# lyndonchan/wsss-analysis

Hardware: AMD Instinct MI355X
Metric: images/sec CAM+CRF pseudo-labels, VOC2012 321x321 (higher is better)
Workload: dtype f16x3; 1 GPU; resnet50 CAM + dense-CRF (M=21, 10 mean-field iters), 321x321, batch 32 images (=64 samples) per GPU, image-sharded; batch_images=32, num_classes=20, parallelism=image-sharded x1, no collective, steps_per_rank=239

## Files before the change

### wsss-analysis_amd/csrc/crf.hip

```cpp
#include "common.h"

#include <atomic>
#include <cmath>
#include <cstring>
#include <memory>

namespace {

constexpr unsigned long long EMPTY_KEY = 0xFFFFFFFFFFFFFFFFull;
typedef float f32x2_t __attribute__((ext_vector_type(2)));

struct LatticeDev {
    int d = 0;
    int rep = 1;
    int rows = 0;
    int32_t *offset = nullptr;
    float *bary = nullptr;
    float *norm = nullptr;
    int2 *nbr = nullptr;
    int32_t *tslot_start = nullptr;
    int2 *slot_desc = nullptr;
    float *tent_w = nullptr;
    uint8_t *tent_p = nullptr;
    int32_t *row_slot_start = nullptr;
    int n_tiles = 0, n_slots = 0;
    bool sorted_dest = false;
    long long n_pix = 0;
    int M_cur = 0;
    float alpha = 0.f;
    int32_t *tile_rows = nullptr;
    int2 *tile_pstart = nullptr;
    int32_t *tile_list = nullptr;
    int n_tiles_occ = 0;
    int4 *gt_cnt = nullptr;
    int2 *gt_rows = nullptr;
    uint4 *gt_nbr = nullptr;
    uint4 *gt_pix = nullptr;
    int gt_stride = 0;
    std::vector<int32_t> v_per_image;
    int32_t *img_row = nullptr;
    int max_img_rows = 0;
    uint32_t *part_row = nullptr;
    bool bl_ok = false;
    int2 *bl_blk = nullptr;
    int bl_cap = 0;
    mutable std::vector<int2> bl_blk_host;
    mutable int bl_M = -1, bl_nblk = 0;
    mutable size_t bl_lds = 0;
};

constexpr int TILE_W = 16, TILE_H = 16, TILE_PIX = TILE_W * TILE_H;
static_assert(TILE_PIX <= 256, "an entry's pixel index is stored in one byte");
constexpr int SLOT_ENT = 32;
constexpr int SORT_MAX = 2048;
static_assert(TILE_PIX * 6 <= SORT_MAX && SORT_MAX <= 65535, "tile too large for the in-LDS grouping");

struct TileGeom {
    int H, W, ntx, nty, tpi;
};
__host__ __device__ inline TileGeom make_geom(int H, int W) {
    TileGeom g;
    g.H = H; g.W = W;
    g.ntx = (W + TILE_W - 1) / TILE_W;
    g.nty = (H + TILE_H - 1) / TILE_H;
    g.tpi = g.ntx * g.nty;
    return g;
}
struct TileBox {
    int x0, y0, cw, ch;
    int ebase;
};
__host__ __device__ inline TileBox tile_box(const TileGeom &g, int j) {
// ... 765 lines not shown
                                                                 float *__restrict__ tent_w, const uint8_t *__restrict__ tent_p) {
    const int tile = blockIdx.x;
    const int b = tile / tg.tpi, j = tile - b * tg.tpi;
    const TileBox tb = tile_box(tg, j);
    const int N = tg.H * tg.W;
    const int ne = tb.cw * tb.ch * dp1;
    const long long ebase = ((long long)b * N + tb.ebase) * dp1;
    const unsigned cw_magic = tile_div_magic(tb.cw);
    for (int i = threadIdx.x; i < ne; i += 256) {
        const int t = (int)tent_p[ebase + i];
        const int ty = (int)(((unsigned)t * cw_magic) >> 16), tx = t - ty * tb.cw;
        const long long p = (long long)b * N + (long long)(tb.y0 + ty) * tg.W + tb.x0 + tx;
        tent_w[ebase + i] = tent_w[ebase + i] * norm[p];
    }
}

template <int D>
__global__ void neighbors_kernel(const unsigned long long *__restrict__ rowkey, const int32_t *__restrict__ rowimg,
                                 const unsigned long long *__restrict__ table, const int32_t *__restrict__ slot2row,
                                 long long cap, unsigned cap_mask, int rows, int2 *__restrict__ nbr) {
    const int j = blockIdx.y;
    long long rbeg, rend;
    xcd_range(rows, rbeg, rend);
    for (int row = (int)rbeg + (int)threadIdx.x; row < (int)rend; row += (int)blockDim.x) {
        const long long i = (long long)j * rows + row;
        int *nb = reinterpret_cast<int *>(nbr);
        if (row == 0) {
            nb[2 * i] = 0;
            continue;
        }
        int key[D], k1[D];
        unpack_key<D>(rowkey[row], key);
#pragma unroll
        for (int k = 0; k < D; ++k) k1[k] = key[k] - 1;
        if (j < D) {
#pragma unroll
            for (int k = 0; k < D; ++k)
                if (k == j) k1[k] = key[k] + D;
        }
        const int b = rowimg[row];
        const unsigned long long *tb = table + (long long)b * cap;
        const int32_t *s2r = slot2row + (long long)b * cap;
        unsigned long long p1;
        int r1 = 0;
        if (pack_key<D>(k1, p1)) {
            const int s = hash_lookup(tb, cap_mask, p1);
            if (s >= 0) r1 = s2r[s];
        }
        nb[2 * i] = r1;
        if (r1 > 0) nb[2 * ((long long)j * rows + r1) + 1] = row;
    }
}


constexpr float PFIX_SCALE = 16777216.0f;
constexpr float PFIX_INV = 1.0f / 16777216.0f;
static_assert(SLOT_ENT * 2.5f < 127.0f, "slot partials must fit the 2^24 fixed-point int32");

template <bool PLAIN>
__device__ __forceinline__ f32x4_t combine_slots4(const f32x4_t *__restrict__ part, int sb, int se, unsigned LP, unsigned l) {
    f32x4_t first = part[(unsigned)sb * LP + l];
    if (se - sb == 1) return first;
    if (PLAIN) {
        for (int i = sb + 1; i < se; ++i) {
            const f32x4_t v = part[(unsigned)i * LP + l];
#pragma unroll
            for (int k = 0; k < 4; ++k) first[k] += v[k];
        }
        return first;
    }
    long long acc[4] = {0, 0, 0, 0};
    for (int i = sb; i < se; i += 4) {
        f32x4_t v[4];
#pragma unroll
        for (int u = 0; u < 4; ++u) v[u] = part[(unsigned)min(i + u, se - 1) * LP + l];
#pragma unroll
        for (int u = 0; u < 4; ++u)
            if (i + u < se) {
#pragma unroll
                for (int k = 0; k < 4; ++k) acc[k] += (long long)__float2int_rn(v[u][k] * PFIX_SCALE);
            }
    }
    f32x4_t o = {(float)acc[0] * PFIX_INV, (float)acc[1] * PFIX_INV, (float)acc[2] * PFIX_INV, (float)acc[3] * PFIX_INV};
    return o;
}

__global__ __launch_bounds__(256) void slot_ones_kernel(const int32_t *__restrict__ tslot_start, const int2 *__restrict__ slot_desc,
                                                        const float *__restrict__ tent_w, int dp1, TileGeom tg,
                                                        float *__restrict__ part) {
    const int tile = blockIdx.x;
    const int b = tile / tg.tpi, j = tile - b * tg.tpi;
    const TileBox tb = tile_box(tg, j);
    const long long ebase = ((long long)b * tg.H * tg.W + tb.ebase) * dp1;
    __shared__ float w[TILE_PIX * 6];
    const int ne = tb.cw * tb.ch * dp1;
    {
        constexpr int EN = (TILE_PIX * 6 + 255) / 256;
        float ew[EN];
#pragma unroll
        for (int k = 0; k < EN; ++k) {
            const int i = (int)threadIdx.x + k * 256;
            ew[k] = i < ne ? tent_w[ebase + i] : 0.f;
        }
#pragma unroll
        for (int k = 0; k < EN; ++k) {
            const int i = (int)threadIdx.x + k * 256;
            if (i < ne) w[i] = ew[k];
        }
    }
    __syncthreads();
    for (int s = tslot_start[tile] + threadIdx.x; s < tslot_start[tile + 1]; s += 256) {
        const int2 d = slot_desc[s];
        const int i0 = d.x & 0xffff, n = d.x >> 16;
        float acc = 0.f;
        for (int i = 0; i < n; ++i) acc += w[i0 + i];
        part[d.y] = acc;
    }
}
__global__ void combine1_kernel(const float *__restrict__ part, const int32_t *__restrict__ row_slot_start, int rows,
                                float *__restrict__ val) {
    for (int row = blockIdx.x * blockDim.x + threadIdx.x; row < rows; row += gridDim.x * blockDim.x) {
        long long acc = 0;
        for (int i = row_slot_start[row]; i < row_slot_start[row + 1]; ++i)
            acc += (long long)__float2int_rn(part[i] * PFIX_SCALE);
        val[row] = (float)acc * PFIX_INV;
    }
}

__global__ __launch_bounds__(256) void combine4_kernel(const f32x4_t *__restrict__ part, const int32_t *__restrict__ row_slot_start,
                                                       int LP, int rows_local, int n_slots, int rep, f32x4_t *__restrict__ val) {
    const int rpb = 256 / LP;
    const int tr = threadIdx.x / LP;
    const int l = threadIdx.x - tr * LP;
    if (tr >= rpb) return;
    long long rbeg, rend;
    int rk;
    xcd_range_rep(rows_local, rep, rk, rbeg, rend);
    part += (size_t)rk * n_slots * LP;
    val += (size_t)rk * rows_local * LP;
    for (long long row = rbeg + tr; row < rend; row += rpb) {
        const int sb = row_slot_start[row], se = row_slot_start[row + 1];
        f32x4_t o = {0.f, 0.f, 0.f, 0.f};
        if (se > sb) o = combine_slots4<true>(part, sb, se, (unsigned)LP, (unsigned)l);
        val[(unsigned)row * (unsigned)LP + l] = o;
    }
}

constexpr int CB_ROWS = 32;
__global__ __launch_bounds__(256) void combine4_balanced_kernel(const f32x4_t *__restrict__ part, const int32_t *__restrict__ row_slot_start,
                                                                const uint32_t *__restrict__ part_row, int LP, int rows,
                                                                f32x4_t *__restrict__ val) {
    __shared__ int rss_l[CB_ROWS + 1];
    __shared__ unsigned long long acc[CB_ROWS * 32];
    const int r0 = blockIdx.x * CB_ROWS;
    const int nr = min(CB_ROWS, rows - r0);
    const int P0 = row_slot_start[r0], P1 = row_slot_start[r0 + nr];
    for (int i = threadIdx.x; i <= nr; i += 256) rss_l[i] = row_slot_start[r0 + i];
    for (int i = threadIdx.x; i < CB_ROWS * 32; i += 256) acc[i] = 0ull;
    const int gpb = 256 / LP;
    const int tr = threadIdx.x / LP, l = threadIdx.x - tr * LP;
    constexpr int U = 4;
    f32x4_t v[U];
    uint32_t pr[U];
    auto fetch = [&](int p) {
#pragma unroll
        for (int u = 0; u < U; ++u) {
            const int pp = p + u * gpb;
            v[u] = f32x4_t{0.f, 0.f, 0.f, 0.f};
            pr[u] = 0u;
            if (tr < gpb && pp < P1) {
                v[u] = part[(unsigned)pp * (unsigned)LP + l];
                if (part_row) pr[u] = part_row[pp];
            }
        }
    };
    fetch(P0 + tr);
    __syncthreads();
    if (tr < gpb) {
        for (int p = P0 + tr; p < P1; p += U * gpb) {
            if (p != P0 + tr) fetch(p);
#pragma unroll
            for (int u = 0; u < U; ++u) {
                const int pp = p + u * gpb;
                if (pp < P1) {
                    int lo;
                    bool single;
                    if (part_row) {
                        lo = (int)(pr[u] & 0xffffffu) - r0;
                        single = (pr[u] >> 24) == 1u;
                    } else {
                        lo = 0;
                        int hi = nr;
                        while (hi - lo > 1) {
                            const int mid = (lo + hi) >> 1;
                            if (rss_l[mid] <= pp) lo = mid;
                            else hi = mid;
                        }
                        single = rss_l[lo + 1] - rss_l[lo] == 1;
                    }
                    if (single) {
                        val[(unsigned)(r0 + lo) * (unsigned)LP + l] = v[u];
                    } else {
#pragma unroll
                        for (int k = 0; k < 4; ++k)
                            atomicAdd(&acc[lo * 32 + 4 * l + k], (unsigned long long)(long long)__float2int_rn(v[u][k] * PFIX_SCALE));
                    }
                }
            }
        }
    }
    __syncthreads();
    if (tr < gpb) {
        for (int row = tr; row < nr; row += gpb) {
            const int n = rss_l[row + 1] - rss_l[row];
            if (n == 1) continue;
            f32x4_t o = {0.f, 0.f, 0.f, 0.f};
            if (n > 1) {
#pragma unroll
                for (int k = 0; k < 4; ++k) o[k] = (float)(long long)acc[row * 32 + 4 * l + k] * PFIX_INV;
            }
            val[(unsigned)(r0 + row) * (unsigned)LP + l] = o;
        }
    }
}


__global__ __launch_bounds__(256) void blur1_kernel(const float *__restrict__ in, const int2 *__restrict__ nbr,
                                                    int rows, float *__restrict__ out) {
    for (int row = blockIdx.x * blockDim.x + threadIdx.x; row < rows; row += gridDim.x * blockDim.x) {
        const int2 nb = nbr[row];
        out[row] = row == 0 ? 0.f : in[row] + 0.5f * (in[nb.x] + in[nb.y]);
    }
}

__global__ __launch_bounds__(256) void blur4_kernel(const f32x4_t *__restrict__ in, const int2 *__restrict__ nbr,
                                                    int LP, int rows_local, int rep, f32x4_t *__restrict__ out) {
    const int rpb = 256 / LP;
    const int tr = threadIdx.x / LP;
    const int l = threadIdx.x - tr * LP;
    if (tr >= rpb) return;
    constexpr int U = 4;
    long long rbeg, rend;
    int rk;
    xcd_range_rep(rows_local, rep, rk, rbeg, rend);
    in += (size_t)rk * rows_local * LP;
    out += (size_t)rk * rows_local * LP;
    for (long long row0 = rbeg + tr; row0 < rend; row0 += U * rpb) {
        int2 nb[U];
        f32x4_t c[U], a[U], b[U];
#pragma unroll
        for (int u = 0; u < U; ++u) {
            const long long row = row0 + u * rpb;
            nb[u] = row < rend ? nbr[row] : make_int2(0, 0);
        }
#pragma unroll
        for (int u = 0; u < U; ++u) {
            const long long row = row0 + u * rpb;
            c[u] = in[(unsigned)(row < rend ? row : 0) * (unsigned)LP + l];
            a[u] = in[(unsigned)nb[u].x * (unsigned)LP + l];
            b[u] = in[(unsigned)nb[u].y * (unsigned)LP + l];
        }
#pragma unroll
        for (int u = 0; u < U; ++u) {
            const long long row = row0 + u * rpb;
            if (row < rend) {
                f32x4_t o;
#pragma unroll
                for (int k = 0; k < 4; ++k) o[k] = row == 0 ? 0.f : c[u][k] + 0.5f * (a[u][k] + b[u][k]);
                out[(unsigned)row * (unsigned)LP + l] = o;
            }
        }
    }
}

constexpr int BL_THREADS = 1024;
constexpr int BL_NVAR = 5;
constexpr int BL_VAR[BL_NVAR][2] = {{4, 4}, {4, 10}, {3, 13}, {2, 20}, {1, 26}};
inline int blur_lds_variant(int rows) {
    for (int v = 0; v < BL_NVAR; ++v)
        if (rows <= BL_VAR[v][1] * BL_THREADS && (size_t)(rows + 1) * BL_VAR[v][0] * 4 <= 160 * 1024 && rows < 65535) return v;
    return -1;
}
struct BlurLdsArgs {
    const int2 *nbr;
    const int32_t *img_row;
    const int2 *blk;
    float *val;
    int Mp, M, rows, npass;
};
template <int GW> struct FloatRun { float v[GW]; };
typedef float f32x3u_t __attribute__((ext_vector_type(3), aligned(4)));
template <int GW>
__device__ __forceinline__ FloatRun<GW> load_run(const float *q) {
    FloatRun<GW> r;
    if constexpr (GW == 4) {
        const f32x4_t x = *reinterpret_cast<const f32x4_t *>(q);
        r.v[0] = x[0]; r.v[1] = x[1]; r.v[2] = x[2]; r.v[3] = x[3];
    } else if constexpr (GW == 3) {
        const f32x3u_t x = *reinterpret_cast<const f32x3u_t *>(q);
        r.v[0] = x[0]; r.v[1] = x[1]; r.v[2] = x[2];
    } else if constexpr (GW == 2) {
        const f32x2_t x = *reinterpret_cast<const f32x2_t *>(q);
        r.v[0] = x[0]; r.v[1] = x[1];
    } else {
        r.v[0] = q[0];
    }
    return r;
}
template <int GW>
__device__ __forceinline__ void store_run(float *q, const FloatRun<GW> &r) {
    if constexpr (GW == 4) *reinterpret_cast<f32x4_t *>(q) = f32x4_t{r.v[0], r.v[1], r.v[2], r.v[3]};
    else if constexpr (GW == 3) {
        f32x3u_t x;
        x[0] = r.v[0]; x[1] = r.v[1]; x[2] = r.v[2];
        *reinterpret_cast<f32x3u_t *>(q) = x;
    } else if constexpr (GW == 2) *reinterpret_cast<f32x2_t *>(q) = f32x2_t{r.v[0], r.v[1]};
    else q[0] = r.v[0];
}
template <int GW, int RPT>
__device__ __forceinline__ void blur_lds_body(const BlurLdsArgs &p, float *pl, int img, int grp) {
    const int r0 = p.img_row[img], nr = p.img_row[img + 1] - r0;
    const int stride = nr + 1;
    const int c0 = grp * GW;
    const int tid = (int)threadIdx.x;
    float *vb = p.val + (size_t)r0 * p.Mp + c0;
    unsigned nb[RPT];
    auto load_idx = [&](int pass) {
        const int2 *q = p.nbr + (size_t)pass * p.rows + r0;
        constexpr int CH = RPT < 10 ? RPT : 10;
#pragma unroll
        for (int i0 = 0; i0 < RPT; i0 += CH) {
            int2 raw[CH];
#pragma unroll
            for (int i = 0; i < CH; ++i) {
                const int r = tid + (i0 + i) * BL_THREADS;
                raw[i] = (i0 + i < RPT && r < nr) ? q[r] : make_int2(0, 0);
            }
#pragma unroll
            for (int i = 0; i < CH; ++i)
                if (i0 + i < RPT)
                    nb[i0 + i] = (unsigned)(raw[i].x ? raw[i].x - r0 : nr) | ((unsigned)(raw[i].y ? raw[i].y - r0 : nr) << 16);
        }
    };
    load_idx(0);
#pragma unroll
    for (int i = 0; i < RPT; ++i) {
        const int r = tid + i * BL_THREADS;
        if (r < nr) {
            FloatRun<GW> run;
            if (GW == 3 && c0 + GW > p.Mp) {
#pragma unroll
                for (int g = 0; g < GW; ++g) run.v[g] = c0 + g < p.Mp ? vb[(size_t)r * p.Mp + g] : 0.f;
            } else {
                run = load_run<GW>(vb + (size_t)r * p.Mp);
            }
#pragma unroll
            for (int g = 0; g < GW; ++g) pl[g * stride + r] = c0 + g < p.M ? run.v[g] : 0.f;
        }
    }
    if (tid < GW) pl[tid * stride + nr] = 0.f;
    __syncthreads();
    float o[RPT][GW];
    for (int pass = 0; pass < p.npass; ++pass) {
#pragma unroll
        for (int i = 0; i < RPT; ++i) {
            const int r = tid + i * BL_THREADS;
            const int rc = r < nr ? r : nr;
            const int l1 = (int)(nb[i] & 0xffffu), l2 = (int)(nb[i] >> 16);
#pragma unroll
            for (int g = 0; g < GW; ++g) o[i][g] = pl[g * stride + rc] + 0.5f * (pl[g * stride + l1] + pl[g * stride + l2]);
        }
        if (pass + 1 < p.npass) load_idx(pass + 1);
        else break;
        __syncthreads();
#pragma unroll
        for (int i = 0; i < RPT; ++i) {
            const int r = tid + i * BL_THREADS;
            if (r < nr) {
#pragma unroll
                for (int g = 0; g < GW; ++g) pl[g * stride + r] = o[i][g];
            }
        }
        __syncthreads();
    }
#pragma unroll
    for (int i = 0; i < RPT; ++i) {
        const int r = tid + i * BL_THREADS;
        if (r < nr) {
            if (c0 + GW <= p.M) {
                FloatRun<GW> run;
#pragma unroll
                for (int g = 0; g < GW; ++g) run.v[g] = o[i][g];
                store_run<GW>(vb + (size_t)r * p.Mp, run);
            } else {
#pragma unroll
                for (int g = 0; g < GW; ++g)
                    if (c0 + g < p.M) vb[(size_t)r * p.Mp + g] = o[i][g];
            }
        }
    }
}
__global__ __launch_bounds__(BL_THREADS) void blur_lds_kernel(BlurLdsArgs p) {
    extern __shared__ float pl[];
    const int2 w = p.blk[blockIdx.x];
    if (w.x < 0) return;
    const int img = w.x & 0xffffff;
    switch (w.x >> 24) {
    case 0: blur_lds_body<BL_VAR[0][0], BL_VAR[0][1]>(p, pl, img, w.y); break;
    case 1: blur_lds_body<BL_VAR[1][0], BL_VAR[1][1]>(p, pl, img, w.y); break;
    case 2: blur_lds_body<BL_VAR[2][0], BL_VAR[2][1]>(p, pl, img, w.y); break;
    case 3: blur_lds_body<BL_VAR[3][0], BL_VAR[3][1]>(p, pl, img, w.y); break;
    default: blur_lds_body<BL_VAR[4][0], BL_VAR[4][1]>(p, pl, img, w.y); break;
    }
}

constexpr int GTI = 12, GTJ = 12, GBI = GTI + 4, GBJ = GTJ + 4;
constexpr int GLH = 6;

__global__ void gauss_ij_kernel(const unsigned long long *__restrict__ rowkey, int rows, int2 *__restrict__ ij,
                                int *__restrict__ bbox ) {
    for (int row = 1 + blockIdx.x * blockDim.x + threadIdx.x; row < rows; row += gridDim.x * blockDim.x) {
        int key[2];
        unpack_key<2>(rowkey[row], key);
        const int a = 2 * key[0] + key[1], b = key[0] + 2 * key[1];
        if (a % 3 != 0 || b % 3 != 0) atomicOr(&bbox[4], 1);
        const int i = a / 3, j = b / 3;
        ij[row] = make_int2(i, j);
        atomicMin(&bbox[0], i);
        atomicMin(&bbox[1], j);
        atomicMax(&bbox[2], i);
        atomicMax(&bbox[3], j);
    }
}

__global__ void gauss_tile_fill_kernel(const int2 *__restrict__ ij, int rows, int imin, int jmin, int nti, int ntj,
                                       int32_t *__restrict__ tile_rows, int32_t *__restrict__ occ) {
    for (int row = 1 + blockIdx.x * blockDim.x + threadIdx.x; row < rows; row += gridDim.x * blockDim.x) {
        const int i = ij[row].x - imin, j = ij[row].y - jmin;
        occ[(i / GTI) * ntj + j / GTJ] = 1;
        for (int ti = (i - GTI - 1 >= 0 ? (i - GTI - 1) / GTI : 0); ti <= (i + 2) / GTI && ti < nti; ++ti) {
            const int li = i - ti * GTI + 2;
            if (li < 0 || li >= GBI) continue;
            for (int tj = (j - GTJ - 1 >= 0 ? (j - GTJ - 1) / GTJ : 0); tj <= (j + 2) / GTJ && tj < ntj; ++tj) {
                const int lj = j - tj * GTJ + 2;
                if (lj < 0 || lj >= GBJ) continue;
                tile_rows[((long long)ti * ntj + tj) * (GBI * GBJ) + li * GBJ + lj] = row;
            }
        }
    }
}

__global__ void gauss_tile_pstart_kernel(const int32_t *__restrict__ tile_rows, const int32_t *__restrict__ row_slot_start,
                                         long long total, int2 *__restrict__ tile_pstart) {
    for (long long i = (long long)blockIdx.x * blockDim.x + threadIdx.x; i < total; i += (long long)gridDim.x * blockDim.x) {
        const int row = tile_rows[i];
        tile_pstart[i] = row ? make_int2(row_slot_start[row], row_slot_start[row + 1] - row_slot_start[row]) : make_int2(0, 0);
// ... 979 lines not shown
    const int b = blockIdx.y;
    const int n0 = blockIdx.x * TP;
    const int np = min(TP, N - n0);
    const long long ibase = ((long long)b * N + n0) * Mp;
    for (int i = threadIdx.x; i < np * Mp; i += TP) {
        const int n = i / Mp, m = i - n * Mp;
        if (m < M) tile[m * (TP + 1) + n] = q[ibase + i];
    }
    __syncthreads();
    if ((int)threadIdx.x < np) {
        if (q_out)
            for (int m = 0; m < M; ++m)
                q_out[((long long)b * M + m) * N + n0 + threadIdx.x] = tile[m * (TP + 1) + threadIdx.x];
        if (argmax) {
            int best = 0;
            float bv = tile[threadIdx.x];
            for (int m = 1; m < M; ++m) {
                const float v = tile[m * (TP + 1) + threadIdx.x];
                if (v > bv) {
                    bv = v;
                    best = m;
                }
            }
            argmax[(long long)b * N + n0 + threadIdx.x] = best;
        }
    }
}

__global__ void fill_tables_kernel(unsigned long long *__restrict__ table, unsigned *__restrict__ first, long long n) {
    for (long long i = (long long)blockIdx.x * blockDim.x + threadIdx.x; i < n; i += (long long)gridDim.x * blockDim.x) {
        table[i] = EMPTY_KEY;
        first[i] = 0x7fffffffu;
    }
}

inline int grid1d(long long total, int per_block = 256, int cap = 256 * 32) {
    long long g = (total + per_block - 1) / per_block;
    if (g > cap) g = cap;
    if (g < 1) g = 1;
    return (int)g;
}

inline int grid_rep(long long total, int per_block, int rep) {
    const int g = grid1d(total, per_block, 256 * 64);
    return g <= rep ? rep : g / rep * rep;
}

void splat_ones(wsc_ctx *ctx, const LatticeDev &L, const TileGeom &tg, float *val, float *part) {
    hipLaunchKernelGGL(slot_ones_kernel, dim3((unsigned)L.n_tiles), dim3(256), 0, ctx->stream, L.tslot_start, L.slot_desc,
                       L.tent_w, L.d + 1, tg, part);
    hipLaunchKernelGGL(combine1_kernel, dim3(grid1d(L.rows)), dim3(256), 0, ctx->stream, part, L.row_slot_start, L.rows, val);
}

void combine4(wsc_ctx *ctx, hipStream_t st, const LatticeDev &L, const float *part, int LP, float *val) {
    WscKernelTimer timer(ctx, WSC_K_BLUR, ((double)L.n_slots + L.rows) * L.rep * L.M_cur * 4);
    if (L.sorted_dest)
        hipLaunchKernelGGL(combine4_kernel, dim3(grid_rep((long long)L.rows * L.rep, 256 / LP, L.rep)), dim3(256), 0,
                           st, (const f32x4_t *)part, L.row_slot_start, LP, L.rows, L.n_slots, L.rep, (f32x4_t *)val);
    else
        hipLaunchKernelGGL(combine4_balanced_kernel, dim3((unsigned)((L.rows + CB_ROWS - 1) / CB_ROWS)), dim3(256), 0, st,
                           (const f32x4_t *)part, L.row_slot_start, (const uint32_t *)L.part_row, LP, L.rows, (f32x4_t *)val);
}

float *blur_all1(wsc_ctx *ctx, const LatticeDev &L, float *a, float *b) {
    for (int j = 0; j <= L.d; ++j) {
        hipLaunchKernelGGL(blur1_kernel, dim3(grid1d(L.rows)), dim3(256), 0, ctx->stream, a,
                           L.nbr + (long long)j * L.rows, L.rows, b);
        float *t = a; a = b; b = t;
    }
    return a;
}

int blur_lds_prepare(wsc_ctx *ctx, const LatticeDev &L, int M) {
    if (L.rep != 1 || !L.img_row || !L.bl_ok) return WSC_OK;
    const int B = (int)L.v_per_image.size();
    if (L.bl_M != M) {
        std::vector<std::vector<int2>> q(8);
        size_t lds = 0;
        for (int b = 0; b < B; ++b) {
            const int v = blur_lds_variant(L.v_per_image[b]), gw = BL_VAR[v][0];
            lds = std::max(lds, (size_t)(L.v_per_image[b] + 1) * gw * 4);
            for (int g = 0; g * gw < M; ++g) q[b & 7].push_back(make_int2(b | (v << 24), g));
        }
        size_t len = 0;
        for (int x = 0; x < 8; ++x) len = std::max(len, q[x].size());
        std::vector<int2> &h = L.bl_blk_host;
        h.assign(len * 8, make_int2(-1, 0));
        for (int x = 0; x < 8; ++x)
            for (size_t i = 0; i < q[x].size(); ++i) h[i * 8 + x] = q[x][i];
        L.bl_M = -1;
        if ((int)h.size() > L.bl_cap) return WSC_OK;
        WSC_TRY(wsc_ctx_upload_small(ctx, L.bl_blk, h.data(), sizeof(int2) * h.size()));
        L.bl_nblk = (int)h.size();
        L.bl_lds = lds;
        L.bl_M = M;
    }
    return WSC_OK;
}
bool blur_lds(wsc_ctx *ctx, hipStream_t st, const LatticeDev &L, int LP, float *val) {
    const int M = L.M_cur;
    if (!ctx->opt[WSC_OPT_CRF_BLUR_ON_CHIP] || L.rep != 1 || !L.img_row || !L.bl_ok || L.bl_M != M) return false;
    if (L.bl_nblk == 0) return true;
    if (wsc_set_max_dynamic_lds(ctx, reinterpret_cast<const void *>(blur_lds_kernel), 160 * 1024) != WSC_OK) return false;
    BlurLdsArgs ba;
    ba.nbr = L.nbr; ba.img_row = L.img_row; ba.blk = L.bl_blk; ba.val = val; ba.Mp = 4 * LP; ba.M = M; ba.rows = L.rows;
    ba.npass = L.d + 1;
    WscKernelTimer timer(ctx, WSC_K_BLUR, 2.0 * (L.d + 1) * L.rows * M * 4);
    hipLaunchKernelGGL(blur_lds_kernel, dim3((unsigned)L.bl_nblk), dim3(BL_THREADS), L.bl_lds, st, ba);
    return true;
}

float *combine_blur_all4(wsc_ctx *ctx, hipStream_t st, const LatticeDev &L, int LP, const float *part, float *a, float *b) {
    const bool fused_off = !ctx->opt[WSC_OPT_CRF_FUSED_BLUR];
    if (L.d == 2 && L.tile_rows && L.tile_pstart && L.n_tiles_occ > 0 && !fused_off) {
        WscKernelTimer timer(ctx, WSC_K_BLUR, ((double)L.n_slots + L.rows) * L.rep * L.M_cur * 4);
        hipLaunchKernelGGL(blur3_tile_kernel, dim3((unsigned)(L.n_tiles_occ * L.rep)), dim3(GBI * GBJ), 0, st,
                           (const f32x4_t *)nullptr, L.tile_rows, L.tile_list, L.n_tiles_occ, LP, L.rows, L.rep, (f32x4_t *)b,
                           (const f32x4_t *)part, L.tile_pstart, L.n_slots);
        return b;
    }
    combine4(ctx, st, L, part, LP, a);
    if (blur_lds(ctx, st, L, LP, a)) return a;
    for (int j = 0; j <= L.d; ++j) {
        WscKernelTimer timer(ctx, WSC_K_BLUR, 2.0 * L.rows * L.rep * L.M_cur * 4);
        hipLaunchKernelGGL(blur4_kernel, dim3(grid_rep((long long)L.rows * L.rep, (256 / LP) * 4, L.rep)), dim3(256),
                           0, st, (const f32x4_t *)a, L.nbr + (long long)j * L.rows, LP, L.rows, L.rep,
                           (f32x4_t *)b);
        float *t = a; a = b; b = t;
    }
    return a;
}

constexpr int GT_MAX_LOCAL = 1022;
int gauss_fuse_tables(wsc_ctx *ctx, const TileGeom &tg, LatticeDev &L, CtxBlocks &own) {
    const int N = tg.H * tg.W, rows = L.rows, W = tg.W;
    std::vector<int32_t> off((size_t)N * 3), rss((size_t)rows + 1);
    std::vector<float> bary((size_t)N * 3), norm((size_t)N);
    std::vector<int2> nbr((size_t)3 * rows);
    WSC_HIP(hipMemcpyAsync(off.data(), L.offset, sizeof(int32_t) * off.size(), hipMemcpyDeviceToHost, ctx->stream));
    WSC_HIP(hipMemcpyAsync(bary.data(), L.bary, sizeof(float) * bary.size(), hipMemcpyDeviceToHost, ctx->stream));
    WSC_HIP(hipMemcpyAsync(norm.data(), L.norm, sizeof(float) * norm.size(), hipMemcpyDeviceToHost, ctx->stream));
    WSC_HIP(hipMemcpyAsync(rss.data(), L.row_slot_start, sizeof(int32_t) * rss.size(), hipMemcpyDeviceToHost, ctx->stream));
    WSC_HIP(hipMemcpyAsync(nbr.data(), L.nbr, sizeof(int2) * nbr.size(), hipMemcpyDeviceToHost, ctx->stream));
    WSC_HIP(hipStreamSynchronize(ctx->stream));
    std::vector<int> loc((size_t)rows, -1);
    std::vector<std::vector<int>> sets((size_t)tg.tpi);
    std::vector<int4> cnt((size_t)tg.tpi);
    int nvmax = 0;
    for (int j = 0; j < tg.tpi; ++j) {
        const TileBox tb = tile_box(tg, j);
        std::vector<int> &list = sets[j];
        auto add = [&](int R) {
            if (R > 0 && R < rows && loc[R] < 0) {
                loc[R] = (int)list.size();
                list.push_back(R);
            }
        };
        for (int ty = 0; ty < tb.ch; ++ty)
            for (int tx = 0; tx < tb.cw; ++tx) {
                const size_t n = (size_t)(tb.y0 + ty) * W + tb.x0 + tx;
                for (int r = 0; r < 3; ++r) add(off[n * 3 + r]);
            }
        int4 &c = cnt[j];
        c.x = (int)list.size();
        for (int axis = 2; axis >= 0; --axis) {
            const size_t cur = list.size();
            for (size_t i = 0; i < cur; ++i) {
                const int2 nb = nbr[(size_t)axis * rows + list[i]];
                add(nb.x);
                add(nb.y);
            }
            if (axis == 2) c.y = (int)list.size();
            if (axis == 1) c.z = (int)list.size();
        }
        c.w = (int)list.size();
// ... 174 lines not shown
            L.bl_cap = 8 * ((B + 7) / 8) * 32;
            WSC_TRY(own.alloc(sizeof(int2) * (size_t)L.bl_cap, &L.bl_blk));
        }
    }

    WSC_TRY(tmp.alloc(sizeof(unsigned long long) * L.rows, &rowkey));
    WSC_TRY(tmp.alloc(sizeof(int32_t) * L.rows, &rowimg));
    WSC_TRY(own.alloc(sizeof(int2) * (size_t)dp1 * L.rows, &L.nbr));

    hipLaunchKernelGGL(assign_rows_kernel, grid_tab, dim3(256), 0, ctx->stream, first, table, cap, per_img, bitmap, wprefix, slot2row,
                       rowkey, rowimg);
    {
        int32_t *slot_row;
        unsigned *sums2, *row_nslots, *cursor, *sums3;
        const int nb2 = (L.n_tiles + 1 + SCAN_CHUNK - 1) / SCAN_CHUNK, nb3 = (L.rows + 1 + SCAN_CHUNK - 1) / SCAN_CHUNK;
        WSC_TRY(tmp.alloc(sizeof(unsigned) * (nb2 + 2), &sums2));
        WSC_TRY(tmp.alloc(sizeof(unsigned) * 2 * (size_t)(L.rows + 1), &row_nslots));
        cursor = row_nslots + (L.rows + 1);
        WSC_TRY(tmp.alloc(sizeof(unsigned) * (nb3 + 2), &sums3));
        WSC_TRY(own.alloc(sizeof(int32_t) * (L.n_tiles + 2), &L.tslot_start));
        WSC_TRY(own.alloc(sizeof(int32_t) * (L.rows + 2), &L.row_slot_start));
        WSC_HIP(hipMemsetAsync(row_nslots, 0, sizeof(unsigned) * 2 * (size_t)(L.rows + 1), ctx->stream));
        WSC_TRY(exclusive_scan(ctx, tile_nslots, L.n_tiles + 1, (unsigned *)L.tslot_start, sums2));
        unsigned ns = 0;
        WSC_HIP(hipMemcpyAsync(&ns, sums2 + nb2, sizeof(unsigned), hipMemcpyDeviceToHost, ctx->stream));
        WSC_HIP(hipStreamSynchronize(ctx->stream));
        L.n_slots = (int)ns;
        WSC_TRY(own.alloc(sizeof(int2) * (size_t)(L.n_slots + 1), &L.slot_desc));
        WSC_TRY(tmp.alloc(sizeof(int32_t) * (size_t)(L.n_slots + 1), &slot_row));
        unsigned *slot_key = nullptr;
        int32_t *dest_slot = nullptr;
        if (D == 2) {
            WSC_TRY(tmp.alloc(sizeof(unsigned) * (size_t)(L.n_slots + 1), &slot_key));
            WSC_TRY(tmp.alloc(sizeof(int32_t) * (size_t)(L.n_slots + 1), &dest_slot));
        }
        hipLaunchKernelGGL(tile_slots_kernel, dim3((unsigned)L.n_tiles), dim3(256), 0, ctx->stream, sslot, L.tent_p, L.offset, slot2row,
                           cap, dp1, tg,
                           L.tslot_start, L.slot_desc, slot_row, slot_key, row_nslots);
        WSC_TRY(exclusive_scan(ctx, row_nslots, L.rows + 1, (unsigned *)L.row_slot_start, sums3));
        if (!shared) WSC_TRY(own.alloc(sizeof(uint32_t) * (size_t)(L.n_slots + 1), &L.part_row));
        hipLaunchKernelGGL(slot_dest_kernel, dim3(grid1d(L.n_slots)), dim3(256), 0, ctx->stream, slot_row, L.n_slots,
                           L.row_slot_start, cursor, L.slot_desc, L.part_row);
        if (D == 2) {
            hipLaunchKernelGGL(dest_inverse_kernel, dim3(grid1d(L.n_slots)), dim3(256), 0, ctx->stream, L.slot_desc, L.n_slots,
                               dest_slot);
            hipLaunchKernelGGL(row_sort_dest_kernel, dim3(grid1d(L.rows)), dim3(256), 0, ctx->stream, slot_key, dest_slot,
                               L.row_slot_start, L.rows, L.slot_desc);
            L.sorted_dest = true;
        }
    }
    WSC_HIP(hipMemsetAsync(L.nbr, 0, sizeof(int2) * (size_t)dp1 * L.rows, ctx->stream));
    hipLaunchKernelGGL(neighbors_kernel<D>, dim3((unsigned)grid1d(L.rows, 256, 4096), (unsigned)dp1), dim3(256), 0, ctx->stream, rowkey,
                       rowimg, table, slot2row, cap, (unsigned)(cap - 1), L.rows, L.nbr);
    WSC_HIP(hipGetLastError());
    if (D == 2) {
        int2 *ij;
        int *bbox;
        WSC_TRY(tmp.alloc(sizeof(int2) * L.rows, &ij));
        WSC_TRY(tmp.alloc(sizeof(int) * 5, &bbox));
        const int init[5] = {0x7fffffff, 0x7fffffff, -0x7fffffff, -0x7fffffff, 0};
        WSC_TRY(wsc_ctx_upload_small(ctx, bbox, init, sizeof(init)));
        hipLaunchKernelGGL(gauss_ij_kernel, dim3(grid1d(L.rows)), dim3(256), 0, ctx->stream, rowkey, L.rows, ij, bbox);
        int hb[5] = {0, 0, -1, -1, 1};
        WSC_HIP(hipMemcpyAsync(hb, bbox, sizeof(hb), hipMemcpyDeviceToHost, ctx->stream));
        WSC_HIP(hipStreamSynchronize(ctx->stream));
        const long long nti = hb[2] >= hb[0] ? ((long long)hb[2] - hb[0]) / GTI + 1 : 0;
        const long long ntj = hb[3] >= hb[1] ? ((long long)hb[3] - hb[1]) / GTJ + 1 : 0;
        if (hb[4] == 0 && nti > 0 && ntj > 0 && nti * ntj <= 4ll * L.rows + 64) {
            const long long nt = nti * ntj;
            int32_t *occ;
            WSC_TRY(tmp.alloc(sizeof(int32_t) * nt, &occ));
            WSC_TRY(own.alloc(sizeof(int32_t) * nt * GBI * GBJ, &L.tile_rows));
            WSC_HIP(hipMemsetAsync(L.tile_rows, 0, sizeof(int32_t) * nt * GBI * GBJ, ctx->stream));
            WSC_HIP(hipMemsetAsync(occ, 0, sizeof(int32_t) * nt, ctx->stream));
            hipLaunchKernelGGL(gauss_tile_fill_kernel, dim3(grid1d(L.rows)), dim3(256), 0, ctx->stream, ij, L.rows, hb[0],
                               hb[1], (int)nti, (int)ntj, L.tile_rows, occ);
            std::vector<int32_t> hocc(nt), list;
            WSC_HIP(hipMemcpyAsync(hocc.data(), occ, sizeof(int32_t) * nt, hipMemcpyDeviceToHost, ctx->stream));
            WSC_HIP(hipStreamSynchronize(ctx->stream));
            for (long long t = 0; t < nt; ++t)
                if (hocc[t]) list.push_back((int32_t)t);
            L.n_tiles_occ = (int)list.size();
            if (L.n_tiles_occ > 0) {
                WSC_TRY(own.alloc(sizeof(int32_t) * list.size(), &L.tile_list));
                WSC_HIP(hipMemcpyAsync(L.tile_list, list.data(), sizeof(int32_t) * list.size(), hipMemcpyHostToDevice,
                                       ctx->stream));
                WSC_HIP(hipStreamSynchronize(ctx->stream));
                WSC_TRY(own.alloc(sizeof(int2) * nt * GBI * GBJ, &L.tile_pstart));
                hipLaunchKernelGGL(gauss_tile_pstart_kernel, dim3(grid1d(nt * GBI * GBJ)), dim3(256), 0, ctx->stream,
                                   L.tile_rows, L.row_slot_start, nt * GBI * GBJ, L.tile_pstart);
            }
        }
    }
    float *va, *vb, *vp;
    WSC_TRY(tmp.alloc(sizeof(float) * L.rows, &va));
    WSC_TRY(tmp.alloc(sizeof(float) * L.rows, &vb));
    WSC_TRY(tmp.alloc(sizeof(float) * (size_t)(L.n_slots + 1), &vp));
    splat_ones(ctx, L, make_geom(crf->H, crf->W), va, vp);
    float *res = blur_all1(ctx, L, va, vb);
    uint32_t *rec_b = nullptr;
    if (D == 5 && !shared && crf->lat[0].gt_rows && !crf->pix_rec_b) WSC_TRY(own.alloc(sizeof(uint32_t) * 13 * (size_t)npix, &rec_b));
    if (!shared && D == 5) {
        hipLaunchKernelGGL(slice_norm_tile_kernel, dim3((unsigned)L.n_tiles), dim3(256), 0, ctx->stream, L.offset, L.bary, dp1,
                           L.alpha, res, make_geom(crf->H, crf->W), L.norm, rec_b, L.tent_w, L.tent_p);
    } else {
        hipLaunchKernelGGL(slice_norm_kernel, dim3(grid1d(npix)), dim3(256), 0, ctx->stream, L.offset, L.bary, dp1,
// ... 206 lines not shown
    if (!crf || M < 1 || M > 32) return 0;
    return update_gf_ok(crf->ctx, crf->lat[0], (M + 3) / 4) ? 1 : 0;
}

static int crf_inference_impl(wsc_ctx *ctx, wsc_crf *crf, const float *unary_dev, bool pixel_major, int M, float g_compat,
                              float bi_compat, int n_iters, float *q_dev, int32_t *argmax_dev);

int wsc_crf_inference(wsc_ctx *ctx, wsc_crf *crf, const float *unary_dev, int M, float g_compat, float bi_compat,
                      int n_iters, float *q_dev, int32_t *argmax_dev) {
    return crf_inference_impl(ctx, crf, unary_dev, false, M, g_compat, bi_compat, n_iters, q_dev, argmax_dev);
}

int wsc_crf_inference_pm(wsc_ctx *ctx, wsc_crf *crf, const float *unary_pm_dev, int M, float g_compat, float bi_compat,
                         int n_iters, float *q_dev, int32_t *argmax_dev) {
    return crf_inference_impl(ctx, crf, unary_pm_dev, true, M, g_compat, bi_compat, n_iters, q_dev, argmax_dev);
}

static int crf_inference_impl(wsc_ctx *ctx, wsc_crf *crf, const float *unary_dev, bool pixel_major, int M, float g_compat,
                              float bi_compat, int n_iters, float *q_dev, int32_t *argmax_dev) {
    WSC_CHECK(ctx && crf && unary_dev, WSC_ERR_INVALID, "wsc_crf_inference: null argument");
    WSC_CHECK(M >= 1 && M <= 32, WSC_ERR_INVALID, "wsc_crf_inference: M=%d outside [1,32]", M);
    WSC_CHECK(n_iters >= 0, WSC_ERR_INVALID, "wsc_crf_inference: n_iters=%d", n_iters);
    WSC_HIP(hipSetDevice(ctx->device));
    const int B = crf->B, N = crf->N;
    const long long npix = (long long)B * N;
    const LatticeDev &G = crf->lat[0], &Bl = crf->lat[1];
    const int LP = (M + 3) / 4, Mp = 4 * LP;
    const long long g_rows = (long long)G.rows * G.rep, g_slots = (long long)G.n_slots * G.rep;
    WSC_CHECK(npix * Mp < (1ll << 30) && g_rows * Mp < (1ll << 30) && (long long)Bl.rows * Mp < (1ll << 30) &&
                  g_slots * Mp < (1ll << 30) && (long long)Bl.n_slots * Mp < (1ll << 30) && npix * 80 < (1ll << 32),
              WSC_ERR_CAPACITY, "CRF batch too large for 32-bit byte offsets (B*N*Mp = %lld elements; split the batch)", npix * Mp);
    WSC_CHECK(N < (1 << 24) && G.rows < (1 << 24) && Bl.rows < (1 << 24), WSC_ERR_CAPACITY,
              "CRF image / lattice too large for 24-bit row arithmetic (N = %d, rows = %d / %d)", N, G.rows, Bl.rows);
    auto al = [](size_t v) { return (v + 255) / 256 * 256; };
    const size_t qb = al(sizeof(float) * npix * Mp);
    const size_t pg = al(sizeof(float) * (size_t)g_slots * Mp), pb = al(sizeof(float) * (size_t)Bl.n_slots * Mp);
    const size_t vg = al(sizeof(float) * (size_t)g_rows * Mp), vb = al(sizeof(float) * (size_t)Bl.rows * Mp);
    void *ws;
    WSC_TRY(wsc_ctx_workspace(ctx, 2 * qb + 2 * vg + 2 * vb + 2 * pg + pb, &ws));
    char *p = (char *)ws;
    float *u = (float *)p; p += qb;
    float *q = (float *)p; p += qb;
    float *vg0 = (float *)p; p += vg;
    float *vg1 = (float *)p; p += vg;
    float *vb0 = (float *)p; p += vb;
    float *vb1 = (float *)p; p += vb;
    float *partg = (float *)p; p += pg;
    float *partg2 = (float *)p; p += pg;
    float *partb = (float *)p; p += pb;

    crf->lat[0].M_cur = M;
    crf->lat[1].M_cur = M;
    if (n_iters > 0) WSC_TRY(blur_lds_prepare(ctx, crf->lat[1], M));
    const dim3 tgrid((N + TP - 1) / TP, B);
    if (!pixel_major) {
        WscKernelTimer timer(ctx, WSC_K_CRF_MISC, (double)npix * M * 12);
        hipLaunchKernelGGL(init_q_kernel, tgrid, dim3(TP), 2 * (size_t)M * (TP + 1) * sizeof(float), ctx->stream,
                           unary_dev, M, Mp, N, u, n_iters == 0 ? q : (float *)nullptr);
    } else {
        u = const_cast<float *>(unary_dev);
    }
    const bool lds_blur = Bl.bl_ok && Bl.img_row && ctx->opt[WSC_OPT_CRF_BLUR_ON_CHIP];
    const bool no_fork = lds_blur || ctx->profiling;
    if (!no_fork && !ctx->aux_stream) {
        WSC_HIP(hipStreamCreateWithFlags(&ctx->aux_stream, hipStreamNonBlocking));
        WSC_HIP(hipEventCreateWithFlags(&ctx->fork_ev, hipEventDisableTiming));
        WSC_HIP(hipEventCreateWithFlags(&ctx->aux_done_ev, hipEventDisableTiming));
    }
    const bool gf = update_gf_ok(ctx, G, LP);
    const bool fg = gf && update_fg_ok(ctx, G, LP) && update_fg_lds_limit(ctx, LP, G.gt_stride) == WSC_OK;
    if (n_iters > 0) WSC_TRY(gf ? crf_bilateral_records(crf, ctx->stream) : crf_full_records(crf, ctx->stream));
    UpdateArgs a = update_args(crf, M, g_compat, bi_compat, u, partg, partb);
    const GaussMsgArgs gm = gauss_msg_args(crf, M, g_compat, partg, u, q);
    const double gf_bytes = 2.0 * 3.0 * (double)(G.rows - 1) * G.rep * M * 4 + (double)npix * (3 * 8 + 1.0 * M * 4);
    if (n_iters == 0 && pixel_major) {
        a.q = q;
        WSC_TRY(launch_update(ctx, a, false, false, false));
    }
    for (int it = 0; it <= n_iters && n_iters > 0; ++it) {
        const bool last = it == n_iters;
        const bool labels_only = last && q_dev == nullptr && argmax_dev != nullptr;
        a.q = last && !labels_only ? q : nullptr;
        a.argmax = labels_only ? argmax_dev : nullptr;
        a.u = (gf && !fg && it > 0) ? q : u;
        if (fg) {
            a.part_g_in = (it & 1) ? partg : partg2;
            a.sg.part = (it & 1) ? partg2 : partg;
        }
        WSC_TRY(launch_update(ctx, a, it > 0, !last, gf, fg && it > 0, gf_bytes));
        if (last) break;
        const bool fork = !no_fork;
        hipStream_t main_stream = ctx->stream;
        if (fork) {
            WSC_HIP(hipEventRecord(ctx->fork_ev, main_stream));
            WSC_HIP(hipStreamWaitEvent(ctx->aux_stream, ctx->fork_ev, 0));
        }
        a.val_b = combine_blur_all4(ctx, fork ? ctx->aux_stream : main_stream, Bl, LP, partb, vb0, vb1);
        if (fork) WSC_HIP(hipEventRecord(ctx->aux_done_ev, ctx->aux_stream));
        if (fg) {
        } else if (gf) WSC_TRY(launch_gauss_msg(ctx, main_stream, gm, gf_bytes));
        else a.val_g = combine_blur_all4(ctx, main_stream, G, LP, partg, vg0, vg1);
        if (fork) WSC_HIP(hipStreamWaitEvent(main_stream, ctx->aux_done_ev, 0));
    }
    {
        WscKernelTimer ftimer(ctx, WSC_K_CRF_MISC, (double)npix * M * 8);
        if (q_dev || (argmax_dev && n_iters == 0))
// ... 135 lines not shown
```

Before: 2645 images/s.

## Write combine output as per-image channel planes and precompute local blur neighbor indices

The balanced combine kernel gains a planar mode. It stages single-slot and accumulated values in LDS with a padded stride, then writes each image's lattice values channel-major so the on-chip blur kernel can load coalesced per-channel planes instead of strided row-major gathers. Neighbor indices are converted once at lattice build time into packed 16-bit image-local offsets, which removes the per-iteration int2 load and conversion. The LDS layout in the blur switches to interleaved GW-wide runs so each neighbor fetch is a vector load. This costs an extra planes buffer, a memset for padded channels, and a binary search per combine block.

```diff
diff --git a/wsss-analysis_amd/csrc/crf.hip b/wsss-analysis_amd/csrc/crf.hip
--- a/wsss-analysis_amd/csrc/crf.hip
+++ b/wsss-analysis_amd/csrc/crf.hip
@@ -18,6 +18,7 @@
     float *bary = nullptr;
     float *norm = nullptr;
     int2 *nbr = nullptr;
+    uint32_t *nbr_local = nullptr;
     int32_t *tslot_start = nullptr;
     int2 *slot_desc = nullptr;
     float *tent_w = nullptr;
@@ -889,6 +890,24 @@
     }
 }
 
+__global__ __launch_bounds__(256) void nbr_local_kernel(const int2 *__restrict__ nbr, const int32_t *__restrict__ rowimg,
+                                                        const int32_t *__restrict__ img_row, int rows, int npass,
+                                                        uint32_t *__restrict__ nbr_local) {
+    for (int row = blockIdx.x * blockDim.x + threadIdx.x; row < rows; row += gridDim.x * blockDim.x) {
+        int r0 = 0, nr = 0;
+        if (row > 0) {
+            const int b = rowimg[row];
+            r0 = img_row[b];
+            nr = img_row[b + 1] - r0;
+        }
+        for (int j = 0; j < npass; ++j) {
+            const size_t i = (size_t)j * rows + row;
+            const int2 nb = nbr[i];
+            nbr_local[i] = row == 0 ? 0u : (unsigned)(nb.x ? nb.x - r0 : nr) | ((unsigned)(nb.y ? nb.y - r0 : nr) << 16);
+        }
+    }
+}
+
 
 constexpr float PFIX_SCALE = 16777216.0f;
 constexpr float PFIX_INV = 1.0f / 16777216.0f;
@@ -984,16 +1003,19 @@
 }
 
 constexpr int CB_ROWS = 32;
+template <bool PLANAR>
 __global__ __launch_bounds__(256) void combine4_balanced_kernel(const f32x4_t *__restrict__ part, const int32_t *__restrict__ row_slot_start,
                                                                 const uint32_t *__restrict__ part_row, int LP, int rows,
-                                                                f32x4_t *__restrict__ val) {
+                                                                f32x4_t *__restrict__ val, const int32_t *__restrict__ img_row,
+                                                                int n_img, float *__restrict__ planes) {
+    constexpr int AS = PLANAR ? 33 : 32;
     __shared__ int rss_l[CB_ROWS + 1];
-    __shared__ unsigned long long acc[CB_ROWS * 32];
+    __shared__ unsigned long long acc[CB_ROWS * AS];
     const int r0 = blockIdx.x * CB_ROWS;
     const int nr = min(CB_ROWS, rows - r0);
     const int P0 = row_slot_start[r0], P1 = row_slot_start[r0 + nr];
     for (int i = threadIdx.x; i <= nr; i += 256) rss_l[i] = row_slot_start[r0 + i];
-    for (int i = threadIdx.x; i < CB_ROWS * 32; i += 256) acc[i] = 0ull;
+    for (int i = threadIdx.x; i < CB_ROWS * AS; i += 256) acc[i] = 0ull;
     const int gpb = 256 / LP;
     const int tr = threadIdx.x / LP, l = threadIdx.x - tr * LP;
     constexpr int U = 4;
@@ -1012,6 +1034,25 @@
         }
     };
     fetch(P0 + tr);
+    const int srow = (int)threadIdx.x & (CB_ROWS - 1);
+    int ir = 0, nrb = 0;
+    if (PLANAR) {
+        int b = 0, hi = n_img;
+        while (hi - b > 1) {
+            const int mid = (b + hi) >> 1;
+            if (img_row[mid] <= r0) b = mid;
+            else hi = mid;
+        }
+        ir = img_row[b];
+        const int e0 = img_row[b + 1];
+        nrb = e0 - ir;
+        if (srow < nr && r0 + srow >= e0) {
+            ++b;
+            while (r0 + srow >= img_row[b + 1]) ++b;
+            ir = img_row[b];
+            nrb = img_row[b + 1] - ir;
+        }
+    }
     __syncthreads();
     if (tr < gpb) {
         for (int p = P0 + tr; p < P1; p += U * gpb) {
@@ -1036,17 +1077,37 @@
                         single = rss_l[lo + 1] - rss_l[lo] == 1;
                     }
                     if (single) {
-                        val[(unsigned)(r0 + lo) * (unsigned)LP + l] = v[u];
+                        if (PLANAR) {
+#pragma unroll
+                            for (int k = 0; k < 4; ++k) acc[lo * AS + 4 * l + k] = (unsigned long long)__float_as_uint(v[u][k]);
+                        } else {
+                            val[(unsigned)(r0 + lo) * (unsigned)LP + l] = v[u];
+                        }
                     } else {
 #pragma unroll
                         for (int k = 0; k < 4; ++k)
-                            atomicAdd(&acc[lo * 32 + 4 * l + k], (unsigned long long)(long long)__float2int_rn(v[u][k] * PFIX_SCALE));
+                            atomicAdd(&acc[lo * AS + 4 * l + k], (unsigned long long)(long long)__float2int_rn(v[u][k] * PFIX_SCALE));
                     }
                 }
             }
         }
     }
     __syncthreads();
+    if (PLANAR) {
+        const int row = srow, gr = r0 + row, Mp = 4 * LP;
+        if (row >= nr) return;
+        if (gr == 0) {
+            for (int c = (int)threadIdx.x / CB_ROWS; c < Mp; c += 256 / CB_ROWS) reinterpret_cast<float *>(val)[c] = 0.f;
+            return;
+        }
+        const int n = rss_l[row + 1] - rss_l[row];
+        float *q = planes + (size_t)ir * Mp + (gr - ir);
+        for (int c = (int)threadIdx.x / CB_ROWS; c < Mp; c += 256 / CB_ROWS) {
+            const unsigned long long a = acc[row * AS + c];
+            q[(size_t)c * nrb] = n == 1 ? __uint_as_float((unsigned)a) : n > 1 ? (float)(long long)a * PFIX_INV : 0.f;
+        }
+        return;
+    }
     if (tr < gpb) {
         for (int row = tr; row < nr; row += gpb) {
             const int n = rss_l[row + 1] - rss_l[row];
@@ -1054,7 +1115,7 @@
             f32x4_t o = {0.f, 0.f, 0.f, 0.f};
             if (n > 1) {
 #pragma unroll
-                for (int k = 0; k < 4; ++k) o[k] = (float)(long long)acc[row * 32 + 4 * l + k] * PFIX_INV;
+                for (int k = 0; k < 4; ++k) o[k] = (float)(long long)acc[row * AS + 4 * l + k] * PFIX_INV;
             }
             val[(unsigned)(r0 + row) * (unsigned)LP + l] = o;
         }
@@ -1119,16 +1180,27 @@
     return -1;
 }
 struct BlurLdsArgs {
-    const int2 *nbr;
+    const uint32_t *nbr_local;
     const int32_t *img_row;
     const int2 *blk;
+    const float *planes;
     float *val;
     int Mp, M, rows, npass;
 };
 template <int GW> struct FloatRun { float v[GW]; };
 typedef float f32x3u_t __attribute__((ext_vector_type(3), aligned(4)));
 template <int GW>
-__device__ __forceinline__ FloatRun<GW> load_run(const float *q) {
+__device__ __forceinline__ void store_run(float *q, const FloatRun<GW> &r) {
+    if constexpr (GW == 4) *reinterpret_cast<f32x4_t *>(q) = f32x4_t{r.v[0], r.v[1], r.v[2], r.v[3]};
+    else if constexpr (GW == 3) {
+        f32x3u_t x;
+        x[0] = r.v[0]; x[1] = r.v[1]; x[2] = r.v[2];
+        *reinterpret_cast<f32x3u_t *>(q) = x;
+    } else if constexpr (GW == 2) *reinterpret_cast<f32x2_t *>(q) = f32x2_t{r.v[0], r.v[1]};
+    else q[0] = r.v[0];
+}
+template <int GW>
+__device__ __forceinline__ FloatRun<GW> get_run(const float *q) {
     FloatRun<GW> r;
     if constexpr (GW == 4) {
         const f32x4_t x = *reinterpret_cast<const f32x4_t *>(q);
@@ -1144,58 +1216,40 @@
     }
     return r;
 }
-template <int GW>
-__device__ __forceinline__ void store_run(float *q, const FloatRun<GW> &r) {
-    if constexpr (GW == 4) *reinterpret_cast<f32x4_t *>(q) = f32x4_t{r.v[0], r.v[1], r.v[2], r.v[3]};
-    else if constexpr (GW == 3) {
-        f32x3u_t x;
-        x[0] = r.v[0]; x[1] = r.v[1]; x[2] = r.v[2];
-        *reinterpret_cast<f32x3u_t *>(q) = x;
-    } else if constexpr (GW == 2) *reinterpret_cast<f32x2_t *>(q) = f32x2_t{r.v[0], r.v[1]};
-    else q[0] = r.v[0];
-}
 template <int GW, int RPT>
 __device__ __forceinline__ void blur_lds_body(const BlurLdsArgs &p, float *pl, int img, int grp) {
     const int r0 = p.img_row[img], nr = p.img_row[img + 1] - r0;
-    const int stride = nr + 1;
     const int c0 = grp * GW;
     const int tid = (int)threadIdx.x;
     float *vb = p.val + (size_t)r0 * p.Mp + c0;
     unsigned nb[RPT];
     auto load_idx = [&](int pass) {
-        const int2 *q = p.nbr + (size_t)pass * p.rows + r0;
-        constexpr int CH = RPT < 10 ? RPT : 10;
-#pragma unroll
-        for (int i0 = 0; i0 < RPT; i0 += CH) {
-            int2 raw[CH];
-#pragma unroll
-            for (int i = 0; i < CH; ++i) {
-                const int r = tid + (i0 + i) * BL_THREADS;
-                raw[i] = (i0 + i < RPT && r < nr) ? q[r] : make_int2(0, 0);
-            }
-#pragma unroll
-            for (int i = 0; i < CH; ++i)
-                if (i0 + i < RPT)
-                    nb[i0 + i] = (unsigned)(raw[i].x ? raw[i].x - r0 : nr) | ((unsigned)(raw[i].y ? raw[i].y - r0 : nr) << 16);
+        const uint32_t *q = p.nbr_local + (size_t)pass * p.rows + r0;
+#pragma unroll
+        for (int i = 0; i < RPT; ++i) {
+            const int r = tid + i * BL_THREADS;
+            nb[i] = r < nr ? q[r] : (unsigned)nr * 0x10001u;
         }
     };
     load_idx(0);
-#pragma unroll
-    for (int i = 0; i < RPT; ++i) {
-        const int r = tid + i * BL_THREADS;
-        if (r < nr) {
-            FloatRun<GW> run;
-            if (GW == 3 && c0 + GW > p.Mp) {
-#pragma unroll
-                for (int g = 0; g < GW; ++g) run.v[g] = c0 + g < p.Mp ? vb[(size_t)r * p.Mp + g] : 0.f;
-            } else {
-                run = load_run<GW>(vb + (size_t)r * p.Mp);
-            }
-#pragma unroll
-            for (int g = 0; g < GW; ++g) pl[g * stride + r] = c0 + g < p.M ? run.v[g] : 0.f;
-        }
-    }
-    if (tid < GW) pl[tid * stride + nr] = 0.f;
+    const float *pb = p.planes + (size_t)r0 * p.Mp + (size_t)c0 * nr;
+#pragma unroll
+    for (int g = 0; g < GW; ++g) {
+        const bool live = c0 + g < p.M;
+        const float *pg = pb + (live ? (size_t)g * nr : 0);
+        float t[RPT];
+#pragma unroll
+        for (int i = 0; i < RPT; ++i) {
+            const int r = tid + i * BL_THREADS;
+            t[i] = r < nr ? pg[r] : 0.f;
+        }
+#pragma unroll
+        for (int i = 0; i < RPT; ++i) {
+            const int r = tid + i * BL_THREADS;
+            if (r < nr) pl[r * GW + g] = live ? t[i] : 0.f;
+        }
+    }
+    if (tid < GW) pl[nr * GW + tid] = 0.f;
     __syncthreads();
     float o[RPT][GW];
     for (int pass = 0; pass < p.npass; ++pass) {
@@ -1204,8 +1258,9 @@
             const int r = tid + i * BL_THREADS;
             const int rc = r < nr ? r : nr;
             const int l1 = (int)(nb[i] & 0xffffu), l2 = (int)(nb[i] >> 16);
-#pragma unroll
-            for (int g = 0; g < GW; ++g) o[i][g] = pl[g * stride + rc] + 0.5f * (pl[g * stride + l1] + pl[g * stride + l2]);
+            const FloatRun<GW> xc = get_run<GW>(pl + rc * GW), x1 = get_run<GW>(pl + l1 * GW), x2 = get_run<GW>(pl + l2 * GW);
+#pragma unroll
+            for (int g = 0; g < GW; ++g) o[i][g] = xc.v[g] + 0.5f * (x1.v[g] + x2.v[g]);
         }
         if (pass + 1 < p.npass) load_idx(pass + 1);
         else break;
@@ -1214,8 +1269,10 @@
         for (int i = 0; i < RPT; ++i) {
             const int r = tid + i * BL_THREADS;
             if (r < nr) {
-#pragma unroll
-                for (int g = 0; g < GW; ++g) pl[g * stride + r] = o[i][g];
+                FloatRun<GW> run;
+#pragma unroll
+                for (int g = 0; g < GW; ++g) run.v[g] = o[i][g];
+                store_run<GW>(pl + r * GW, run);
             }
         }
         __syncthreads();
@@ -1238,7 +1295,7 @@
     }
 }
 __global__ __launch_bounds__(BL_THREADS) void blur_lds_kernel(BlurLdsArgs p) {
-    extern __shared__ float pl[];
+    extern __shared__ __attribute__((aligned(16))) float pl[];
     const int2 w = p.blk[blockIdx.x];
     if (w.x < 0) return;
     const int img = w.x & 0xffffff;
@@ -2324,14 +2381,20 @@
     hipLaunchKernelGGL(combine1_kernel, dim3(grid1d(L.rows)), dim3(256), 0, ctx->stream, part, L.row_slot_start, L.rows, val);
 }
 
-void combine4(wsc_ctx *ctx, hipStream_t st, const LatticeDev &L, const float *part, int LP, float *val) {
+void combine4(wsc_ctx *ctx, hipStream_t st, const LatticeDev &L, const float *part, int LP, float *val, float *planes = nullptr) {
     WscKernelTimer timer(ctx, WSC_K_BLUR, ((double)L.n_slots + L.rows) * L.rep * L.M_cur * 4);
+    const dim3 cb_grid((unsigned)((L.rows + CB_ROWS - 1) / CB_ROWS));
     if (L.sorted_dest)
         hipLaunchKernelGGL(combine4_kernel, dim3(grid_rep((long long)L.rows * L.rep, 256 / LP, L.rep)), dim3(256), 0,
                            st, (const f32x4_t *)part, L.row_slot_start, LP, L.rows, L.n_slots, L.rep, (f32x4_t *)val);
+    else if (planes)
+        hipLaunchKernelGGL(combine4_balanced_kernel<true>, cb_grid, dim3(256), 0, st, (const f32x4_t *)part, L.row_slot_start,
+                           (const uint32_t *)L.part_row, LP, L.rows, (f32x4_t *)val, (const int32_t *)L.img_row,
+                           (int)L.v_per_image.size(), planes);
     else
-        hipLaunchKernelGGL(combine4_balanced_kernel, dim3((unsigned)((L.rows + CB_ROWS - 1) / CB_ROWS)), dim3(256), 0, st,
-                           (const f32x4_t *)part, L.row_slot_start, (const uint32_t *)L.part_row, LP, L.rows, (f32x4_t *)val);
+        hipLaunchKernelGGL(combine4_balanced_kernel<false>, cb_grid, dim3(256), 0, st, (const f32x4_t *)part, L.row_slot_start,
+                           (const uint32_t *)L.part_row, LP, L.rows, (f32x4_t *)val, (const int32_t *)nullptr, 0,
+                           (float *)nullptr);
 }
 
 float *blur_all1(wsc_ctx *ctx, const LatticeDev &L, float *a, float *b) {
@@ -2369,17 +2432,19 @@
     }
     return WSC_OK;
 }
-bool blur_lds(wsc_ctx *ctx, hipStream_t st, const LatticeDev &L, int LP, float *val) {
-    const int M = L.M_cur;
-    if (!ctx->opt[WSC_OPT_CRF_BLUR_ON_CHIP] || L.rep != 1 || !L.img_row || !L.bl_ok || L.bl_M != M) return false;
-    if (L.bl_nblk == 0) return true;
-    if (wsc_set_max_dynamic_lds(ctx, reinterpret_cast<const void *>(blur_lds_kernel), 160 * 1024) != WSC_OK) return false;
+bool blur_lds_ok(wsc_ctx *ctx, const LatticeDev &L) {
+    if (!ctx->opt[WSC_OPT_CRF_BLUR_ON_CHIP] || L.rep != 1 || !L.img_row || !L.nbr_local || !L.bl_ok || L.bl_M != L.M_cur ||
+        L.bl_nblk == 0)
+        return false;
+    return wsc_set_max_dynamic_lds(ctx, reinterpret_cast<const void *>(blur_lds_kernel), 160 * 1024) == WSC_OK;
+}
+void blur_lds(wsc_ctx *ctx, hipStream_t st, const LatticeDev &L, int LP, const float *planes, float *val) {
     BlurLdsArgs ba;
-    ba.nbr = L.nbr; ba.img_row = L.img_row; ba.blk = L.bl_blk; ba.val = val; ba.Mp = 4 * LP; ba.M = M; ba.rows = L.rows;
+    ba.nbr_local = L.nbr_local; ba.img_row = L.img_row; ba.blk = L.bl_blk; ba.planes = planes; ba.val = val; ba.Mp = 4 * LP;
+    ba.M = L.M_cur; ba.rows = L.rows;
     ba.npass = L.d + 1;
-    WscKernelTimer timer(ctx, WSC_K_BLUR, 2.0 * (L.d + 1) * L.rows * M * 4);
+    WscKernelTimer timer(ctx, WSC_K_BLUR, 2.0 * (L.d + 1) * L.rows * L.M_cur * 4);
     hipLaunchKernelGGL(blur_lds_kernel, dim3((unsigned)L.bl_nblk), dim3(BL_THREADS), L.bl_lds, st, ba);
-    return true;
 }
 
 float *combine_blur_all4(wsc_ctx *ctx, hipStream_t st, const LatticeDev &L, int LP, const float *part, float *a, float *b) {
@@ -2391,8 +2456,12 @@
                            (const f32x4_t *)part, L.tile_pstart, L.n_slots);
         return b;
     }
+    if (blur_lds_ok(ctx, L)) {
+        combine4(ctx, st, L, part, LP, a, b);
+        blur_lds(ctx, st, L, LP, b, a);
+        return a;
+    }
     combine4(ctx, st, L, part, LP, a);
-    if (blur_lds(ctx, st, L, LP, a)) return a;
     for (int j = 0; j <= L.d; ++j) {
         WscKernelTimer timer(ctx, WSC_K_BLUR, 2.0 * L.rows * L.rep * L.M_cur * 4);
         hipLaunchKernelGGL(blur4_kernel, dim3(grid_rep((long long)L.rows * L.rep, (256 / LP) * 4, L.rep)), dim3(256),
@@ -2673,6 +2742,11 @@
     WSC_HIP(hipMemsetAsync(L.nbr, 0, sizeof(int2) * (size_t)dp1 * L.rows, ctx->stream));
     hipLaunchKernelGGL(neighbors_kernel<D>, dim3((unsigned)grid1d(L.rows, 256, 4096), (unsigned)dp1), dim3(256), 0, ctx->stream, rowkey,
                        rowimg, table, slot2row, cap, (unsigned)(cap - 1), L.rows, L.nbr);
+    if (!shared && L.bl_ok) {
+        WSC_TRY(own.alloc(sizeof(uint32_t) * (size_t)dp1 * L.rows, &L.nbr_local));
+        hipLaunchKernelGGL(nbr_local_kernel, dim3((unsigned)grid1d(L.rows)), dim3(256), 0, ctx->stream, (const int2 *)L.nbr,
+                           (const int32_t *)rowimg, (const int32_t *)L.img_row, L.rows, dp1, L.nbr_local);
+    }
     WSC_HIP(hipGetLastError());
     if (D == 2) {
         int2 *ij;
@@ -2985,6 +3059,7 @@
     crf->lat[0].M_cur = M;
     crf->lat[1].M_cur = M;
     if (n_iters > 0) WSC_TRY(blur_lds_prepare(ctx, crf->lat[1], M));
+    if (n_iters > 0 && Mp != M && blur_lds_ok(ctx, Bl)) WSC_HIP(hipMemsetAsync(vb0, 0, sizeof(float) * (size_t)Bl.rows * Mp, ctx->stream));
     const dim3 tgrid((N + TP - 1) / TP, B);
     if (!pixel_major) {
         WscKernelTimer timer(ctx, WSC_K_CRF_MISC, (double)npix * M * 12);
```

Result: no change. 2640 images/s (-0.2%).
